# kevinzakka/mink

Hardware: AMD Instinct MI355X
Metric: IK solves/sec (whole node), Unitree G1 4 FrameTasks + box limits, batch 65536 (higher is better)
Workload: dtype f64

## Files before the change

### mink_amd/csrc/build.py

```python

import concurrent.futures
import json
import os
import re
import shutil
import subprocess
import sys
from typing import NamedTuple

HERE = os.path.dirname(os.path.abspath(__file__))
PKG = os.path.dirname(HERE)
_TAG = os.environ.get("MKH_BUILD_TAG", "")
LIB = os.path.join(PKG, f"libminkhip_{_TAG}.so" if _TAG else "libminkhip.so")
RESOURCES = os.path.join(PKG, f"kernel_resources_{_TAG}.json" if _TAG else "kernel_resources.json")
BUILD = os.path.join(HERE, f"_build_{_TAG}" if _TAG else "_build")
def _sources() -> list:
    fs = [os.path.join(HERE, f) for f in sorted(os.listdir(HERE))
          if f.endswith((".h", ".hip", ".py", ".inc")) and f not in ("tab_asm.inc", "__init__.py")]
    return fs + [os.path.join(HERE, "..", "..", "include", "minkhip.h")]


NTS = (8, 16, 24, 32, 44, 48, 64)
FEATS = (0, 16, 6, 8, 72, 88, 136, 30, 31, 256)
WOOD = ((16, 16), (24, 24), (32, 32), (44, 44), (48, 48))
W3 = ((44, 0),)
W3_WOOD = ((44, 44, 32), (44, 44, 48), (32, 32, 32), (32, 32, 48),
           (24, 24, 32), (24, 24, 48), (16, 16, 32), (16, 16, 48),
           (44, 44, 36), (44, 44, 52))
W3_WOOD_ONE_SHOT = ((44, 44, 32), (44, 44, 32, "w4"))
WOOD_FEATS = (32, 48, 33, 36, 52)
WOOD_ROWS = ((48, 48, 40),)


class Variant(NamedTuple):
    nt: int
    feat: int
    nr: int = 0
    w3: bool = False
    one_shot: bool = False
    w4 = False

    @property
    def name(self) -> str:
        return f"{self.nt}_{self.feat}" + (f"_r{self.nr}" if self.nr else "") + (("_w4" if self.w4 else "_w3") if self.w3 else "") + ("o" if self.one_shot else "")

    def translation_unit(self) -> str:
        defs = [f"MKH_NT {self.nt}"] + ([f"MKH_NR {self.nr}"] if self.nr else []) + [f"MKH_FEAT {self.feat}"]
        if self.w3:
            defs.append("MKH_W3 1")
            if self.w4:
                defs.append("MKH_W4P 1")
            elif self.nr and self.nt <= 24 and not self.one_shot:
                defs.append("MKH_W4 1")
        if self.one_shot:
            defs.append("MKH_ONE_SHOT 1")
        if self.name != f"{self.nt}_{self.feat}":
            defs.append(f"MKH_KERNEL_NAME ik_solve_kernel_{self.name}")
        return "// generated by build.py\n" + "".join(f"#define {d}\n" for d in defs) + f"""#include "../ik_kernel.h"
namespace mkh {{
void launch_{self.name}(int grid, int lds_bytes, hipStream_t stream, const DeviceProblem* P, const SolveArgs& a,
                      const TapArgs* taps) {{
  hipLaunchKernelGGL(ik_solve_kernel_{self.name}, dim3(grid), dim3(kWave), lds_bytes, stream, P, a, taps);
}}
}}  // namespace mkh
"""


class VariantW4(Variant):
    __slots__ = ()
    w4 = True


VARIANTS = tuple([Variant(nt, ft) for nt in NTS for ft in FEATS]
                 + [Variant(nt, ft, nr) for nt, nr in WOOD for ft in WOOD_FEATS]
                 + [Variant(nt, ft, nr) for nt, nr, ft in WOOD_ROWS]
                 + [Variant(nt, ft, w3=True) for nt, ft in W3]
                 + [Variant(nt, ft, nr, w3=True) for nt, nr, ft in W3_WOOD]
                 + [(VariantW4 if e[3:] == ("w4",) else Variant)(e[0], e[2], e[1], w3=True, one_shot=True) for e in W3_WOOD_ONE_SHOT])
FLAGS = ["--offload-arch=gfx950", "-O3", "-std=c++17", "-fPIC", "-Wno-unused-result", "-Wno-null-conversion"]
FLAGS += os.environ.get("MKH_EXTRA_FLAGS", "").split()
KERNEL_FLAGS = ["-mllvm", "-disable-machine-licm",
                "-Wno-inline-asm"]


def _hipcc() -> str:
    return shutil.which("hipcc") or "/opt/rocm/bin/hipcc"


def _stale() -> bool:
    if not os.path.exists(LIB) or not os.path.exists(RESOURCES) or not os.path.exists(BUILD_INFO):
        return True
    t = os.path.getmtime(LIB)
    return any(os.path.getmtime(p) > t for p in _sources()) \
        or not os.path.exists(os.path.join(HERE, "tab_asm.inc"))


def _deps(depfile: str) -> list:
    txt = open(depfile).read().replace("\\\n", " ")
    return [d for d in txt.split(":", 1)[1].split() if d]


def _obj_stale(src: str, obj: str, cmd_tag: str) -> bool:
    dep, tag = obj + ".d", obj + ".cmd"
    if not (os.path.exists(obj) and os.path.exists(dep) and os.path.exists(tag)) or open(tag).read() != cmd_tag:
        return True
    t = os.path.getmtime(obj)
    try:
        return any(os.path.getmtime(d) > t for d in [src] + _deps(dep))
    except OSError:
        return True


def _parse_resource_remarks(stderr: str) -> dict:
    out, cur = {}, None
    keys = {"VGPRs": "vgprs", "AGPRs": "agprs", "TotalSGPRs": "sgprs", "ScratchSize [bytes/lane]": "scratch_bytes_per_lane",
            "Occupancy [waves/SIMD]": "occupancy_waves_per_simd", "SGPRs Spill": "sgpr_spills", "VGPRs Spill": "vgpr_spills"}
    for m in re.finditer(r"remark:\s+([A-Za-z \[\]/]+): (\S+) \[-Rpass-analysis", stderr):
        k, v = m.group(1).strip(), m.group(2)
        if k == "Function Name":
            cur = out.setdefault(v, {})
        elif cur is not None and k in keys:
            cur[keys[k]] = int(v)
    return out


def _short_name(mangled: str) -> str:
    m = re.match(r"_ZN(?:3mkh|12_GLOBAL__N_1)(\d+)", mangled)
    if not m:
        return mangled
    n, a = int(m.group(1)), m.end()
    name, rest = mangled[a:a + n], mangled[a + n:]
    if rest.startswith("I"):
        args = re.match(r"I((?:L[ib]\d+E)+)E", rest)
        if args:
            name += "<" + ",".join(re.findall(r"L[ib](\d+)E", args.group(1))) + ">"
    return name


def _sha256(path: str) -> str:
    import hashlib
    h = hashlib.sha256()
    with open(path, "rb") as fh:
        for blk in iter(lambda: fh.read(1 << 20), b""):
            h.update(blk)
    return h.hexdigest()


def _device_code_sha256(obj: str) -> str:
    import hashlib
    import tempfile
    llvm = "/opt/rocm/lib/llvm/bin"
    try:
        with tempfile.TemporaryDirectory() as d:
            fat, co = os.path.join(d, "x.fatbin"), os.path.join(d, "x.co")
            subprocess.run([f"{llvm}/llvm-objcopy", f"--dump-section=.hip_fatbin={fat}", obj, os.path.join(d, "x.o")], check=True, capture_output=True)
            subprocess.run([f"{llvm}/clang-offload-bundler", "--unbundle", "--type=o", "--targets=hipv4-amdgcn-amd-amdhsa--gfx950",
                            f"--input={fat}", f"--output={co}"], check=True, capture_output=True)
            h = hashlib.sha256()
            for sec in (".text", ".rodata"):
                out = os.path.join(d, "sec.bin")
                subprocess.run([f"{llvm}/llvm-objcopy", "-O", "binary", f"--only-section={sec}", co, out], check=True, capture_output=True)
                with open(out, "rb") as fh:
                    h.update(fh.read())
            return h.hexdigest()
    except (OSError, subprocess.CalledProcessError):
        return _sha256(obj)


def _git_state() -> dict:
    root = os.path.dirname(PKG)
    try:
        head = subprocess.run(["git", "-C", root, "rev-parse", "HEAD"], capture_output=True, text=True, check=True).stdout.strip()
        dirty = subprocess.run(["git", "-C", root, "status", "--porcelain", "--", "mink_amd", "include"], capture_output=True,
                               text=True, check=True).stdout.strip() != ""
        return {"git_head": head, "git_dirty_sources": dirty}
    except (OSError, subprocess.CalledProcessError):
        return {"git_head": None, "git_dirty_sources": None}


BUILD_INFO = os.path.join(PKG, f"build_info_{_TAG}.json" if _TAG else "build_info.json")


def _write_resources(objs: list) -> None:
    table = {}
    for o in objs:
        path = o + ".res.json"
        if not os.path.exists(path):
            continue
        fns = json.load(open(path))
        kernels = {f: r for f, r in fns.items() if "ik_solve_kernel" in f or "ik_lane_kernel" in f or "_kernel" in _short_name(f)}
        callees = {f: r for f, r in fns.items() if f not in kernels}
        code = _device_code_sha256(o)
        for f, r in kernels.items():
            e = dict(r)
            e["code_sha256"] = code
            e["callees"] = {_short_name(c): cr for c, cr in callees.items()}
            e["vgpr_spills_with_callees"] = r.get("vgpr_spills", 0) + sum(cr.get("vgpr_spills", 0) for cr in callees.values())
            e["sgpr_spills_with_callees"] = r.get("sgpr_spills", 0) + sum(cr.get("sgpr_spills", 0) for cr in callees.values())
            table[_short_name(f)] = e
    with open(RESOURCES, "w") as fh:
        json.dump(table, fh, indent=0, sort_keys=True)
    info = {"library": os.path.basename(LIB), "library_sha256": _sha256(LIB)}
    info.update(_git_state())
    with open(BUILD_INFO, "w") as fh:
# ... 111 lines not shown
```

### mink_amd/csrc/ik_kernel.h

```cpp
#pragma once
#include "collide_dev.h"
#include "lds_layout.h"
#include "lie_dev.h"
#include "mkh_types.h"
#include "wave_ops.h"
#include "tab_asm.inc"
#include <utility>

#if defined(MKH_W4P) && !defined(MKH_W4)
#define MKH_W4 1
#endif
#if defined(MKH_W4)
#define MKH_TAB TabW4
#elif defined(MKH_W3)
#define MKH_TAB TabW3
#else
#define MKH_TAB Tab
#endif

#if defined(MKH_W3) || (defined(MKH_FEAT) && (MKH_FEAT & 8) && !(MKH_FEAT & 1) && !(MKH_FEAT & 64) && (!(MKH_FEAT & 128) || !defined(MKH_INLINE_136)))
#define MKH_CALLS 1
#endif

namespace mkh {
// ... 155 lines not shown
  const double2 a = o[0], b = o[1];
  ps.d = a.x; ps.sg = a.y; ps.x = b.x; ps.rn = b.y;
  if (FULL) {
    const double2 c = o[2];
    ps.lo = c.x; ps.hi = c.y;
  }
  double rowv = 0.0;
#ifdef MKH_W4P
  rowv = MKH_TAB<NT>::row_on_demand_1(ts, p0, p1, col, npiv, lds_addr(sPiv + kPivBuf));
#else
  if constexpr (MKH_TAB<NT>::kHist > 0) rowv = MKH_TAB<NT>::row_on_demand(ts, p0, p1, col, npiv);
#endif
  return (lane == col || lane >= nact) ? 0.0 : rowv;
}
template <int NT>
__device__ __forceinline__ void load_factor_column(typename MKH_TAB<NT>::Regs& ts, const double* sJ, const double* sDinv, int lane, int n_mu) {
  if constexpr (MKH_TAB<NT>::kHist > 0) MKH_TAB<NT>::load_gz(ts, lds_addr(sJ + (lane < NT ? lane : 0)), lds_addr(sDinv), n_mu);
}
#ifdef MKH_W4P
#define MKH_HS_PARAM , double* sHs
#define MKH_HS_ARG , sPiv + kPivBuf
#else
#define MKH_HS_PARAM
#define MKH_HS_ARG
#endif
template <int NT>
__device__ __forceinline__ void pivot_product(typename MKH_TAB<NT>::Regs& ts, QpLane& s, int k, bool reverse, int lane, double own,
                                              const PivotScalars& ps, double inv, int& npiv MKH_HS_PARAM) {
  const double sk = ps.sg;
  const double ck = s.sg * sk * own;
#ifdef MKH_W4P
  MKH_TAB<NT>::hist_push_1(ts, npiv, own);
  if (lane == k) reinterpret_cast<double2*>(sHs)[npiv] = double2{sk * sk, inv};
#else
  const double g = (sk * sk) * own * inv;
  if constexpr (MKH_TAB<NT>::kHist > 0) MKH_TAB<NT>::hist_push(ts, npiv, -g, own);
#endif
  ++npiv;
  if (lane == k) {
    s.D = -inv;
    s.sg = (reverse ? -sk : sk) * inv;
  } else {
    s.D = fma(-ck * inv, ck, s.D);
  }
}

constexpr bool kTapIsProf_t_xpos = false, kTapIsProf_t_xquat = false, kTapIsProf_t_frame_pose = false,
               kTapIsProf_t_subtree_com = false, kTapIsProf_t_task_e = false, kTapIsProf_t_task_J = false,
               kTapIsProf_t_H = false, kTapIsProf_t_c = false, kTapIsProf_t_box_lo = false, kTapIsProf_t_box_hi = false,
               kTapIsProf_t_coll_G = false, kTapIsProf_t_coll_h = false, kTapIsProf_t_qp_iters = true,
               kTapIsProf_t_cycles = true;


#ifdef MKH_NT
#ifdef MKH_DEBUG_ALL_TAPS
#define MKH_TAP(f) ((kTaps && tp) ? tp->f : nullptr)
#else
#define MKH_TAP(f) ((kTaps && tp && (!kWood || kTapIsProf_##f)) ? tp->f : nullptr)
#endif
#define MKH_CAT2(a, b, c) a##b##_##c
#define MKH_CAT(a, b, c) MKH_CAT2(a, b, c)
#ifndef MKH_KERNEL_NAME
#define MKH_KERNEL_NAME MKH_CAT(ik_solve_kernel_, MKH_NT, MKH_FEAT)
#endif

#ifdef MKH_MARKERS
#define MKH_MARK(name) asm volatile("; MKH_MARK " name)
#else
#define MKH_MARK(name) do {} while (0)
#endif

struct PreOut { int status, d_kind, d_k, d_body, d_qadr, conv; double mu_lane; V3 com_root; };
#ifdef MKH_CALLS
#ifdef MKH_ONE_SHOT
#define MKH_PRE_ATTR __attribute__((noinline, internal_linkage))
#else
#define MKH_PRE_ATTR __attribute__((noinline))
#endif
#ifdef MKH_CLOCKS
#define MKH_PRE_TC_PARAMS , long long* clk_row
#define MKH_PRE_TC_ARGS , (A.clk ? A.clk + (size_t)pb * 24 + 20 : nullptr)
#define MKH_PRE_TICK() do { if (clk_row) { *clk_row = __builtin_readcyclecounter(); ++clk_row; } asm volatile("" : "+v"(lane)); } while (0)
#define MKH_PRE_STOP(id) do { if (clk_row_stop == (id)) return PreOut{}; } while (0)
#else
#define MKH_PRE_TC_PARAMS
#define MKH_PRE_TC_ARGS
#define MKH_PRE_TICK() do { asm volatile("" : "+v"(lane)); } while (0)
#define MKH_PRE_STOP(id) do {} while (0)
#endif
#else
#define MKH_PRE_ATTR __forceinline__
#define MKH_PRE_TC_PARAMS , long long (&tc)[8], int& tci
#define MKH_PRE_TC_ARGS , tc, tci
#ifdef MKH_CLOCKS
#define MKH_PRE_TICK() do { tc[tci] = __builtin_readcyclecounter(); ++tci; asm volatile("" : "+v"(lane)); } while (0)
#else
#define MKH_PRE_TICK() do { if (MKH_TAP(t_cycles)) tc[tci] = __builtin_readcyclecounter(); ++tci; asm volatile("" : "+v"(lane)); } while (0)
#endif
#define MKH_PRE_STOP(id) do {} while (0)
#endif
#define MKH_GLOBAL __attribute__((address_space(1)))
#define MKH_CONSTANT __attribute__((address_space(4)))
struct PreView {
  const MKH_GLOBAL double *body_f, *jnt_f, *dof_f;
  const MKH_GLOBAL int32_t *body_i, *jnt_i, *dof_i;
  const MKH_GLOBAL FrameTaskDev* frame;
  int nbody, nv, nq, njnt, n_frame, n_posture, n_com, max_rows, n_jrows, prefetch, prefetch_w3, prefetch_w3w, wood_compact, prefetch_wc, n_rows_tap, nrounds, robot_root, n_hsel, jnt_pos_zero;
  __device__ __forceinline__ explicit PreView(const DeviceProblem* Pq) {
    const MKH_CONSTANT DeviceProblem* c = (const MKH_CONSTANT DeviceProblem*)Pq;
    body_f = (const MKH_GLOBAL double*)c->body_f; jnt_f = (const MKH_GLOBAL double*)c->jnt_f; dof_f = (const MKH_GLOBAL double*)c->dof_f;
    body_i = (const MKH_GLOBAL int32_t*)c->body_i; jnt_i = (const MKH_GLOBAL int32_t*)c->jnt_i; dof_i = (const MKH_GLOBAL int32_t*)c->dof_i;
    frame = (const MKH_GLOBAL FrameTaskDev*)c->frame;
    nbody = c->nbody; nv = c->nv; nq = c->nq; njnt = c->njnt; n_frame = c->n_frame; n_posture = c->n_posture; n_com = c->n_com;
    max_rows = c->max_rows; n_jrows = c->n_jrows; prefetch = c->prefetch; prefetch_w3 = c->prefetch_w3; prefetch_w3w = c->prefetch_w3w;
    wood_compact = c->wood_compact; prefetch_wc = c->prefetch_wc;
    n_rows_tap = c->n_rows_tap; nrounds = c->nrounds; robot_root = c->robot_root; n_hsel = c->n_hsel;
    jnt_pos_zero = c->jnt_pos_zero;
  }
};
template <class PT>
__device__ __forceinline__ bool kernel_prefetch(const PT& P0) {
  constexpr bool kWood = (MKH_FEAT & F_WOOD) != 0;
  constexpr bool kWoodRows = kWood && (MKH_FEAT & (F_COLL | F_DENSE)) != 0;
#if defined(MKH_W4P)
  (void)kWood; (void)kWoodRows; (void)P0;
  return false;
#elif defined(MKH_W3)
  return (kWood ? P0.prefetch_w3w : P0.prefetch_w3) != 0;
#else
  return ((kWoodRows || (kWood && P0.wood_compact != 0)) ? P0.prefetch_wc : P0.prefetch) != 0;
#endif
}
#ifdef MKH_NR
#define MKH_LAYOUT_NR MKH_NR
#else
#define MKH_LAYOUT_NR MKH_NT
#endif
#ifdef MKH_W3
#define MKH_LAYOUT_W3 true
#else
#define MKH_LAYOUT_W3 false
#endif
#ifdef MKH_W4P
#define kernel_lds_layout(P0) build_lds_layout_w4p(P0, MKH_LAYOUT_NR)
#else
#define kernel_lds_layout(P0) build_lds_layout(P0, MKH_NT, MKH_LAYOUT_NR, MKH_FEAT, MKH_LAYOUT_W3)
#endif
#ifdef MKH_W4P
#define MKH_PRE_RF_PARAM , int refetch, const SolveArgs* args_p
#define MKH_PRE_RF_ARG , (refac_in ? 1 : 0), (const SolveArgs*)A_p
#else
#define MKH_PRE_RF_PARAM
#define MKH_PRE_RF_ARG
#endif
__device__ MKH_PRE_ATTR PreOut pre_phases(const DeviceProblem* Pq, const TapArgs* tp, int pb, int oz, int off_q, int off_tgt,
                                          bool until, double pos_thr, double ori_thr MKH_PRE_RF_PARAM MKH_PRE_TC_PARAMS) {
  constexpr int FEAT = MKH_FEAT;
  constexpr bool kTaps = (FEAT & F_TAPS) != 0, kRel = (FEAT & F_REL) != 0, kCom = (FEAT & F_COM) != 0;
  constexpr bool kSteps = (FEAT & F_STEPS) != 0, kWood = (FEAT & F_WOOD) != 0;
  extern __shared__ __attribute__((aligned(16))) double smem[];
#if defined(MKH_CALLS) && defined(MKH_CLOCKS)
  const int clk_row_stop = clk_row ? (int)clk_row[-5] : 0;
#endif
#ifdef MKH_CALLS
  pb = uni(pb); oz = uni(oz); off_q = uni(off_q); off_tgt = uni(off_tgt);
  until = uni((int)until) != 0; pos_thr = uni(pos_thr); ori_thr = uni(ori_thr);
  Pq = reinterpret_cast<const DeviceProblem*>(uni((unsigned long long)reinterpret_cast<size_t>(Pq)));
  tp = reinterpret_cast<const TapArgs*>(uni((unsigned long long)reinterpret_cast<size_t>(tp)));
#endif
#ifdef MKH_CALLS
  const PreView P(Pq);
#else
  const DeviceProblem& P = *Pq;
#endif
  int lane = lane_id();
  const int ol = lane + oz;
  const int nbody = P.nbody, nv = P.nv;
  const LdsLayout L = kernel_lds_layout(P);
  double* const sq = smem + off_q;
  double* const sX = smem + L.X;
  const int XS = lds_even(nbody);
  double* const sJnt = smem + L.jnt;
  double* const sTgt = smem + off_tgt;
  double* const sTask = smem + L.task;
  double* const sDof = smem + L.dof;
  double* const sCom = smem + L.com;
  const bool is_body = lane < nbody;
  const bool is_dof = lane < nv;
  int status = 0;
#ifdef MKH_W4P
  if (uni(refetch) != 0) {
    typedef const __attribute__((address_space(1))) void* gptr_t;
    typedef __attribute__((address_space(3))) void* lptr_t;
    const MKH_CONSTANT SolveArgs& A = *(const MKH_CONSTANT SolveArgs*)uni((unsigned long long)reinterpret_cast<size_t>(args_p));
    wave_sync();
    const int ndq = 2 * P.nq, ndt = 2 * P.n_frame * 7;
    const char* gq = reinterpret_cast<const char*>(A.q + (size_t)pb * P.nq);
    for (int b0 = 0; b0 < ndq; b0 += kWave)
      if (b0 + lane < ndq)
        __builtin_amdgcn_global_load_lds((gptr_t)(gq + 4 * (b0 + lane)), (lptr_t)(reinterpret_cast<char*>(sq) + 4 * b0), 4, 0, 0);
    const char* gt = reinterpret_cast<const char*>(A.frame_targets + (size_t)pb * (ndt / 2));
    for (int b0 = 0; b0 < ndt; b0 += kWave)
      if (b0 + lane < ndt)
        __builtin_amdgcn_global_load_lds((gptr_t)(gt + 4 * (b0 + lane)), (lptr_t)(reinterpret_cast<char*>(sTgt) + 4 * b0), 4, 0, 0);
    asm volatile("s_waitcnt vmcnt(0)" ::: "memory");
    wave_sync();
  }
#endif
    V3 xp{0, 0, 0};
    Q4 xq{1, 0, 0, 0};
    int b_jadr = 0, b_jnum = 0, anc_lo = 0, anc_hi = 0;
    const bool jp_zero = kWood && P.jnt_pos_zero != 0;
    if (is_body) {
      anc_lo = P.body_i[BI_ANCPACK0 * 64 + ol];
      anc_hi = P.body_i[BI_ANCPACK1 * 64 + ol];
      const auto* bf = P.body_f + ol;
      xp = {bf[(BF_POS + 0) * 64], bf[(BF_POS + 1) * 64], bf[(BF_POS + 2) * 64]};
      xq = {bf[(BF_QUAT + 0) * 64], bf[(BF_QUAT + 1) * 64], bf[(BF_QUAT + 2) * 64], bf[(BF_QUAT + 3) * 64]};
      b_jadr = P.body_i[BI_JNTADR * 64 + ol];
      b_jnum = P.body_i[BI_JNTNUM * 64 + ol];
      for (int jn = 0; jn < b_jnum; ++jn) {
        const int j = b_jadr + jn;
        const int jt = P.jnt_i[j * JI_COUNT + JI_TYPE];
        const int qa = P.jnt_i[j * JI_COUNT + JI_QADR];
        const auto* jfp = P.jnt_f + j * JF_COUNT;
#ifdef MKH_W4P
        const auto* const jf = jfp;
#else
        const double jf[JF_COUNT] = {jfp[0], jfp[1], jfp[2], jfp[3], jfp[4], jfp[5], jfp[6]};
#endif
        if (jt == JNT_FREE) {
          xp = {sq[qa], sq[qa + 1], sq[qa + 2]};
          xq = qnormalize(Q4{sq[qa + 3], sq[qa + 4], sq[qa + 5], sq[qa + 6]});
        } else if (jt == JNT_SLIDE) {
          V3 ax{jf[JF_AXIS], jf[JF_AXIS + 1], jf[JF_AXIS + 2]};
          xp = xp + (sq[qa] - jf[JF_QPOS0]) * qrot(xq, ax);
        } else {
          V3 jp{jf[JF_POS], jf[JF_POS + 1], jf[JF_POS + 2]};
          Q4 qloc;
          if (jt == JNT_HINGE) {
            V3 ax{jf[JF_AXIS], jf[JF_AXIS + 1], jf[JF_AXIS + 2]};
            qloc = axis_angle(ax, sq[qa] - jf[JF_QPOS0]);
          } else {
            qloc = qnormalize(Q4{sq[qa], sq[qa + 1], sq[qa + 2], sq[qa + 3]});
          }
          V3 anchor = xp;
          if (!jp_zero) anchor = xp + qrot(xq, jp);
          xq = qmul(xq, qloc);
          xp = anchor;
          if (!jp_zero) xp = anchor - qrot(xq, jp);
        }
      }
    }
    for (int r = 0; r < P.nrounds; ++r) {
      wave_sync();
      if (is_body) {
        double* o = sX + lane;
        o[0] = xp.x; o[XS] = xp.y; o[2 * XS] = xp.z; o[3 * XS] = xq.w; o[4 * XS] = xq.x; o[5 * XS] = xq.y; o[6 * XS] = xq.z;
      }
      wave_sync();
      if (is_body) {
        const double* a = sX + (((r < 5) ? (anc_lo >> (6 * r)) : anc_hi) & 63);
        V3 ap{a[0], a[XS], a[2 * XS]};
        Q4 aq{a[3 * XS], a[4 * XS], a[5 * XS], a[6 * XS]};
        xp = ap + qrot(aq, xp);
        xq = qmul(aq, xq);
      }
    }
    xq = qnormalize(xq);
    wave_sync();
    if (is_body) {
      double* o = sX + lane;
      o[0] = xp.x; o[XS] = xp.y; o[2 * XS] = xp.z; o[3 * XS] = xq.w; o[4 * XS] = xq.x; o[5 * XS] = xq.y; o[6 * XS] = xq.z;
      if (MKH_TAP(t_xpos)) {
        double* t = MKH_TAP(t_xpos) + ((size_t)pb * nbody + lane) * 3;
        t[0] = xp.x; t[1] = xp.y; t[2] = xp.z;
      }
      if (MKH_TAP(t_xquat)) {
        double* t = MKH_TAP(t_xquat) + ((size_t)pb * nbody + lane) * 4;
        t[0] = xq.w; t[1] = xq.x; t[2] = xq.y; t[3] = xq.z;
      }
    }
    wave_sync();
    MKH_MARK("fk_done");
    MKH_PRE_TICK();
    MKH_PRE_STOP(1);
    if (is_body && b_jnum > 0) {
      if (b_jnum == 1) {
        const int j = b_jadr;
        const auto* jf = P.jnt_f + j * JF_COUNT;
        V3 ax = qrot(xq, V3{jf[JF_AXIS], jf[JF_AXIS + 1], jf[JF_AXIS + 2]});
        V3 an = xp;
        if (!jp_zero) an = xp + qrot(xq, V3{jf[JF_POS], jf[JF_POS + 1], jf[JF_POS + 2]});
        double* o = sJnt + j * 6;
        o[0] = ax.x; o[1] = ax.y; o[2] = ax.z; o[3] = an.x; o[4] = an.y; o[5] = an.z;
      } else {
        const double* a = sX + P.body_i[BI_PARENT * 64 + ol];
        const auto* bf = P.body_f + ol;
        V3 fp = V3{a[0], a[XS], a[2 * XS]} + qrot(Q4{a[3 * XS], a[4 * XS], a[5 * XS], a[6 * XS]},
                                            V3{bf[(BF_POS + 0) * 64], bf[(BF_POS + 1) * 64], bf[(BF_POS + 2) * 64]});
        Q4 fq = qmul(Q4{a[3 * XS], a[4 * XS], a[5 * XS], a[6 * XS]}, Q4{bf[(BF_QUAT + 0) * 64], bf[(BF_QUAT + 1) * 64],
                                                    bf[(BF_QUAT + 2) * 64], bf[(BF_QUAT + 3) * 64]});
        for (int jn = 0; jn < b_jnum; ++jn) {
          const int j = b_jadr + jn;
          const int jt = P.jnt_i[j * JI_COUNT + JI_TYPE];
          const int qa = P.jnt_i[j * JI_COUNT + JI_QADR];
          const auto* jf = P.jnt_f + j * JF_COUNT;
          V3 axl{jf[JF_AXIS], jf[JF_AXIS + 1], jf[JF_AXIS + 2]};
          V3 jp{jf[JF_POS], jf[JF_POS + 1], jf[JF_POS + 2]};
          V3 ax = qrot(fq, axl);
          V3 an = fp + qrot(fq, jp);
          double* o = sJnt + j * 6;
          o[0] = ax.x; o[1] = ax.y; o[2] = ax.z; o[3] = an.x; o[4] = an.y; o[5] = an.z;
          if (jt == JNT_SLIDE) {
            fp = fp + (sq[qa] - jf[JF_QPOS0]) * ax;
          } else if (jt == JNT_HINGE || jt == JNT_BALL) {
            Q4 qloc = (jt == JNT_HINGE) ? axis_angle(axl, sq[qa] - jf[JF_QPOS0])
                                        : qnormalize(Q4{sq[qa], sq[qa + 1], sq[qa + 2], sq[qa + 3]});
            fq = qmul(fq, qloc);
            fp = an - qrot(fq, jp);
          }
        }
      }
    }
    wave_sync();
    int d_kind = DOF_HINGE, d_k = 0, d_body = 0, d_qadr = -1;
    {
    V3 d_ang{0, 0, 0}, d_lin{0, 0, 0}, d_anchor{0, 0, 0};
    double q_dof = 0.0;
    const double r_lo = P.dof_f[DF_RANGE_LO * 64 + ol], r_hi = P.dof_f[DF_RANGE_HI * 64 + ol];
    if (is_dof) {
      const auto* di = P.dof_i + ol;
      const int d_jnt = di[DI_JNT * 64];
      d_kind = di[DI_KIND * 64];
      d_k = di[DI_K * 64];
      d_body = di[DI_BODY * 64];
      d_qadr = di[DI_QADR * 64];
      if (d_kind == DOF_HINGE) {
        const double* o = sJnt + d_jnt * 6;
        d_ang = {o[0], o[1], o[2]};
        d_anchor = {o[3], o[4], o[5]};
        q_dof = sq[d_qadr];
      } else if (d_kind == DOF_SLIDE) {
        const double* o = sJnt + d_jnt * 6;
        d_lin = {o[0], o[1], o[2]};
        q_dof = sq[d_qadr];
      } else if (d_kind == DOF_FREE_LIN) {
        d_lin = {d_k == 0 ? 1.0 : 0.0, d_k == 1 ? 1.0 : 0.0, d_k == 2 ? 1.0 : 0.0};
      } else {
        const double* xb = sX + d_body;
        M3 R = qmat(Q4{xb[3 * XS], xb[4 * XS], xb[5 * XS], xb[6 * XS]});
        d_ang = (d_k == 0) ? V3{R.m[0], R.m[3], R.m[6]}
                           : ((d_k == 1) ? V3{R.m[1], R.m[4], R.m[7]} : V3{R.m[2], R.m[5], R.m[8]});
        if (d_kind == DOF_FREE_ANG) {
          d_anchor = {xb[0], xb[XS], xb[2 * XS]};
        } else {
          const double* o = sJnt + d_jnt * 6;
          d_anchor = {o[3], o[4], o[5]};
        }
      }
    }
    {
      const bool ball0 = is_dof && d_kind == DOF_BALL && d_k == 0;
      const bool ranged = (is_dof && (d_kind == DOF_HINGE || d_kind == DOF_SLIDE)) || ball0;
      const double qc = ball0 ? sq[ball0 ? d_qadr : 0] : q_dof;
      const bool viol = ranged & ((qc < r_lo - 1e-6) | (qc > r_hi + 1e-6));
      if (__ballot(viol)) status |= 1;
    }
    if (is_dof) {
      double* o = sDof + lane * 10;
      o[0] = d_ang.x; o[1] = d_ang.y; o[2] = d_ang.z; o[3] = d_lin.x; o[4] = d_lin.y; o[5] = d_lin.z;
      o[6] = d_anchor.x; o[7] = d_anchor.y; o[8] = d_anchor.z; o[9] = q_dof;
    }
    }

    V3 com_root{0, 0, 0};
    if (kCom && P.n_com > 0) {
      V3 b_ipos{0, 0, 0};
      double b_mass = 0.0, b_stmass = 0.0;
      int b_last = 0, b_inrobot = 0;
      if (is_body) {
        const auto* bf = P.body_f + ol;
        b_ipos = {bf[(BF_IPOS + 0) * 64], bf[(BF_IPOS + 1) * 64], bf[(BF_IPOS + 2) * 64]};
        b_mass = bf[BF_MASS * 64];
        b_stmass = bf[BF_SUBTREEMASS * 64];
        b_last = P.body_i[BI_SUBTREE_LAST * 64 + ol];
        b_inrobot = P.body_i[BI_IN_ROBOT * 64 + ol];
      }
      V3 xi = xp + qrot(xq, b_ipos);
      const double m = (is_body && b_inrobot) ? b_mass : 0.0;
      double sx = m * xi.x, sy = m * xi.y, sz = m * xi.z;
#pragma unroll
      for (int o = 1; o < 64; o <<= 1) {
        double tx = __shfl_up(sx, o), ty = __shfl_up(sy, o), tz = __shfl_up(sz, o);
        if (lane >= o) { sx += tx; sy += ty; sz += tz; }
      }
      const int hi_l = is_body ? b_last : 0, lo_l = lane - 1;
      double ex = __shfl(sx, hi_l), ey = __shfl(sy, hi_l), ez = __shfl(sz, hi_l);
      double bx = __shfl(sx, lo_l < 0 ? 0 : lo_l), by = __shfl(sy, lo_l < 0 ? 0 : lo_l),
             bz = __shfl(sz, lo_l < 0 ? 0 : lo_l);
      if (lane == 0) { bx = 0; by = 0; bz = 0; }
      V3 cs = xi;
      if (b_stmass >= 1e-15) {
        const double im = fast_rcp(b_stmass);
        cs = {(ex - bx) * im, (ey - by) * im, (ez - bz) * im};
      }
      if (is_body) {
        double* o = sCom + lane * 4;
        o[0] = cs.x; o[1] = cs.y; o[2] = cs.z; o[3] = b_stmass;
      }
      wave_sync();
      const double* cr = sCom + P.robot_root * 4;
      com_root = {cr[0], cr[1], cr[2]};
      if (MKH_TAP(t_subtree_com) && lane < 3) MKH_TAP(t_subtree_com)[(size_t)pb * 3 + lane] = cr[lane];
    }

    MKH_MARK("axes_done");
    MKH_PRE_TICK();
    MKH_PRE_STOP(2);
    double mu_lane = 0.0;
    bool conv_lane = true;
    if (lane < P.n_frame) {
      const auto& ft = P.frame[lane];
      const double* xb = sX + ft.body;
      SE3 F;
      Q4 bq{xb[3 * XS], xb[4 * XS], xb[5 * XS], xb[6 * XS]};
      F.p = V3{xb[0], xb[XS], xb[2 * XS]} + qrot(bq, V3{ft.lpos[0], ft.lpos[1], ft.lpos[2]});
      F.q = qmul(bq, Q4{ft.lquat[0], ft.lquat[1], ft.lquat[2], ft.lquat[3]});
      const double* tg = sTgt + lane * 7;
      SE3 Tt{Q4{tg[0], tg[1], tg[2], tg[3]}, V3{tg[4], tg[5], tg[6]}};
      double* o = sTask + lane * 64;
      V3 ev, ew;
      double Jm[9], Qm[9];
      bool ident;
      double eth = 0.0;
      const double* const eth_p = kWood ? &eth : nullptr;
#ifdef MKH_W4P
      {
        const M3 Rf0 = qmat(F.q);
#pragma unroll
        for (int i = 0; i < 9; ++i) o[18 + i] = Rf0.m[i];
        o[27] = F.p.x; o[28] = F.p.y; o[29] = F.p.z;
      }
#endif
      if (!(kRel && ft.relative)) {
        se3_log(se3_mul(se3_inv(F), Tt), ev, ew, eth);
        se3_ljacinv(ev, ew, eth_p, Jm, Qm, ident);
      } else {
        const double* xr = sX + ft.root_body;
        Q4 rq0{xr[3 * XS], xr[4 * XS], xr[5 * XS], xr[6 * XS]};
        SE3 Rt;
        Rt.p = V3{xr[0], xr[XS], xr[2 * XS]} + qrot(rq0, V3{ft.root_lpos[0], ft.root_lpos[1], ft.root_lpos[2]});
        Rt.q = qmul(rq0, Q4{ft.root_lquat[0], ft.root_lquat[1], ft.root_lquat[2], ft.root_lquat[3]});
        const SE3 Tfr = se3_mul(se3_inv(Rt), F);
        se3_log(se3_mul(se3_inv(Tt), Tfr), ev, ew, eth);
        se3_ljacinv(-1.0 * ev, -1.0 * ew, eth_p, Jm, Qm, ident);
        const SE3 Trf = se3_inv(Tfr);
        const M3 Rr = qmat(Rt.q), Rrf = qmat(Trf.q);
#pragma unroll
        for (int i = 0; i < 9; ++i) { o[36 + i] = Rr.m[i]; o[48 + i] = Rrf.m[i]; }
        o[45] = Rt.p.x; o[46] = Rt.p.y; o[47] = Rt.p.z;
        o[57] = Trf.p.x; o[58] = Trf.p.y; o[59] = Trf.p.z;
        if (MKH_TAP(t_frame_pose)) {
          double* t = MKH_TAP(t_frame_pose) + ((size_t)pb * P.n_frame + lane) * 7;
          t[0] = Tfr.q.w; t[1] = Tfr.q.x; t[2] = Tfr.q.y; t[3] = Tfr.q.z; t[4] = Tfr.p.x; t[5] = Tfr.p.y; t[6] = Tfr.p.z;
        }
      }
#ifdef MKH_W4P
#pragma unroll
      for (int i = 0; i < 9; ++i) { o[i] = Jm[i]; o[9 + i] = Qm[i]; }
#else
      M3 Rf = qmat(F.q);
#pragma unroll
      for (int i = 0; i < 9; ++i) { o[i] = Jm[i]; o[9 + i] = Qm[i]; o[18 + i] = Rf.m[i]; }
      o[27] = F.p.x; o[28] = F.p.y; o[29] = F.p.z;
#endif
      const double e6[6] = {ev.x, ev.y, ev.z, ew.x, ew.y, ew.z};
      double ss = 0.0;
#pragma unroll
      for (int r = 0; r < 6; ++r) {
        const double we = ft.cost[r] * (-ft.gain * e6[r]);
        o[30 + r] = we;
        ss += we * we;
        if (MKH_TAP(t_task_e)) MKH_TAP(t_task_e)[(size_t)pb * P.n_rows_tap + ft.row0 + r] = e6[r];
      }
      mu_lane = ft.lm_damping * ss;
      if (kSteps && until) {
        const double pt = pos_thr, ot = ori_thr;
        conv_lane = (!(ft.rowmask & 7) || dot(ev, ev) <= pt * pt) && (!(ft.rowmask & 56) || dot(ew, ew) <= ot * ot);
      }
      if (MKH_TAP(t_frame_pose) && !(kRel && ft.relative)) {
        double* t = MKH_TAP(t_frame_pose) + ((size_t)pb * P.n_frame + lane) * 7;
        t[0] = F.q.w; t[1] = F.q.x; t[2] = F.q.y; t[3] = F.q.z; t[4] = F.p.x; t[5] = F.p.y; t[6] = F.p.z;
      }
    }
  PreOut po;
  po.status = status; po.d_kind = d_kind; po.d_k = d_k; po.d_body = d_body; po.d_qadr = d_qadr;
  po.conv = conv_lane ? 1 : 0; po.mu_lane = mu_lane; po.com_root = com_root;
  return po;
}

template <bool kRel>
__device__ __forceinline__ void frame_column_fn(const double* sTask, const double* sDof, int t, int k, uint64_t mask,
                                                uint64_t rmask, bool rel, double (&Jt)[6]) {
    const double* o = sTask + t * 64;
    const double* kd = sDof + k * 10;
    const V3 d_ang{kd[0], kd[1], kd[2]}, d_lin{kd[3], kd[4], kd[5]}, d_anchor{kd[6], kd[7], kd[8]};
    V3 a{0, 0, 0}, w{0, 0, 0};
    if ((mask >> k) & 1) {
      V3 pf{o[27], o[28], o[29]};
      V3 jp = d_lin + cross(d_ang, pf - d_anchor);
      M3 Rf;
#pragma unroll
      for (int i = 0; i < 9; ++i) Rf.m[i] = o[18 + i];
      a = mulT(Rf, jp); w = mulT(Rf, d_ang);
    }
    double sign = -1.0;
    if (kRel && rel) {
      sign = 1.0;
      if ((rmask >> k) & 1) {
        V3 pr{o[45], o[46], o[47]};
        V3 jp = d_lin + cross(d_ang, pr - d_anchor);
        M3 Rr, Rrf;
#pragma unroll
        for (int i = 0; i < 9; ++i) { Rr.m[i] = o[36 + i]; Rrf.m[i] = o[48 + i]; }
        V3 ar = mulT(Rr, jp), wr = mulT(Rr, d_ang);
        V3 Rw = mul(Rrf, wr);
        a = a - (mul(Rrf, ar) + cross(V3{o[57], o[58], o[59]}, Rw));
        w = w - Rw;
      }
    }
    const double wv[3] = {w.x, w.y, w.z};
    double y[3], z3[3];
#pragma unroll
    for (int r = 0; r < 3; ++r) y[r] = o[3 * r] * wv[0] + o[3 * r + 1] * wv[1] + o[3 * r + 2] * wv[2];
    const double av[3] = {a.x, a.y, a.z};
#pragma unroll
    for (int r = 0; r < 3; ++r)
      z3[r] = av[r] - (o[9 + 3 * r] * y[0] + o[9 + 3 * r + 1] * y[1] + o[9 + 3 * r + 2] * y[2]);
#pragma unroll
    for (int r = 0; r < 3; ++r) {
      Jt[r] = sign * (o[3 * r] * z3[0] + o[3 * r + 1] * z3[1] + o[3 * r + 2] * z3[2]);
      Jt[3 + r] = sign * y[r];
    }
  }

struct DirectPairs { double Jp[6]; int p_task, p_dof; };
__device__ MKH_PRE_ATTR DirectPairs direct_pairs(const DeviceProblem* Pq) {
  constexpr bool kRel = (MKH_FEAT & F_REL) != 0;
  extern __shared__ __attribute__((aligned(16))) double smem[];
#ifdef MKH_CALLS
  Pq = reinterpret_cast<const DeviceProblem*>(uni((unsigned long long)reinterpret_cast<size_t>(Pq)));
  const MKH_CONSTANT DeviceProblem& P = *(const MKH_CONSTANT DeviceProblem*)Pq;
  const MKH_GLOBAL FrameTaskDev* const frames = (const MKH_GLOBAL FrameTaskDev*)P.frame;
#else
  const DeviceProblem& P = *Pq;
  const FrameTaskDev* const frames = P.frame;
#endif
  const int lane = lane_id();
  const LdsLayout L = kernel_lds_layout(P);
  DirectPairs dp{{0, 0, 0, 0, 0, 0}, -1, 0};
  if (lane < P.n_dpairs) {
    dp.p_task = P.dpair_task[lane]; dp.p_dof = P.dpair_dof[lane];
    const auto& ft = frames[dp.p_task];
    const bool rel = kRel && ft.relative != 0;
    double Jt[6];
    frame_column_fn<kRel>(smem + L.task, smem + L.dof, dp.p_task, dp.p_dof, ft.dof_mask, rel ? ft.root_mask : 0ull, rel, Jt);
#pragma unroll
    for (int r = 0; r < 6; ++r) dp.Jp[r] = ft.cost[r] * Jt[r];
  }
  return dp;
}


#if (MKH_FEAT & 32)
struct WoodOut { double hdiag, dsq, x, D, rown; int status, clamp; };

template <int SRC, int O0, int O1>
__device__ __forceinline__ void wood_store_pivot(unsigned addr, double inv, double om) {
  static_assert(SRC >= 0 && SRC < kWave && O0 >= 0 && O0 < 256 && O1 >= 0 && O1 < 256, "lane / ds_write2 offsets");
  unsigned long long sv;
  asm volatile("s_mov_b64 %[sv], exec\n\ts_lshl_b64 exec, 1, %[src]\n\tds_write2_b64 %[a], %[x], %[y] offset0:%[o0] offset1:%[o1]\n\t"
               "s_mov_b64 exec, %[sv]"
               : [sv] "=&s"(sv) : [a] "v"(addr), [x] "v"(inv), [y] "v"(om), [src] "n"(SRC), [o0] "n"(O0), [o1] "n"(O1) : "memory", "scc");
}

struct WoodRefine { bool on; int nv; double lo, hi, zfree, dsq, sqdg, zsq; };
template <int K, bool DUAL>
__device__ __forceinline__ void wood_eliminate(int n_mu, int NR, int lane, double* sJ, double* sS, int SP, const double* sW,
                                               double* sRow, double* sDinv, double& ssq, double& quad, double& zw, int& status,
                                               const WoodRefine& rf, int& clamp, double& beta) {
  const unsigned plane_off = (unsigned)(lane & 15);
  if constexpr (!DUAL) {
    const int my_c = lane - NR;
    const bool is_s = my_c >= 0 && my_c < n_mu;
    double z[K];
    {
      const double* src = sJ + lane;
      int stride = NR;
      bool live = lane < NR;
      if (is_s) { src = sS + my_c * SP; stride = 1; live = true; }
#pragma unroll
      for (int r = 0; r < K; ++r) z[r] = (live && r < n_mu) ? src[r * stride] : 0.0;
    }
    double ws = is_s ? sW[my_c] : 0.0;
    {
      double q = 0.0;
#pragma unroll
      for (int r = 0; r < K; ++r) q = fma(z[r], z[r], q);
      if (lane < NR) sJ[n_mu * NR + lane] = q;
    }
    double* const sOm = sDinv + kMuOm;
    int n_mu_s = uni(n_mu);
    unsigned dinv_addr = lds_addr(sDinv);
    asm volatile("" : "+v"(dinv_addr));
#pragma nounroll
    for (int pass = 0;; ++pass) {
      quad = 0.0; zw = 0.0;
      asm volatile("" : "+s"(n_mu_s));
      static_for<K>([&](auto rc) {
        constexpr int r = decltype(rc)::value;
        if (r < n_mu_s) {
          const double d = readlane_f64(z[r], NR + r), om = readlane_f64(ws, NR + r);
          const double p0 = bperm_f64(z[r], NR + (int)plane_off);
          const double p1 = (K > 16) ? bperm_f64(z[r], (NR + 16 + (int)plane_off) & 63) : 0.0;
          if (lane < NR) sJ[r * NR + lane] = z[r];
          const double inv = fast_rcp(d);
          wood_store_pivot<(MKH_NT + r) % kWave, r, kMuOm + r>(dinv_addr, inv, ws);
          const double zi = z[r] * inv;
          quad = fma(z[r], zi, quad);
          zw = fma(om, zi, zw);
          WoodElim<r, K>::step(z, p0, p1, -zi);
          ws = fma(-zi, om, ws);
        }
      });
      if (lane < n_mu && !(sDinv[lane] > 0.0)) status |= 4;
      if (pass == 1 || !rf.on) break;
#ifdef MKH_W4P
      double rc = rf.zsq, rd = rf.dsq, rh = rf.sqdg;
      asm volatile("" : "+v"(rc), "+v"(rd), "+v"(rh));
      double rf_zfree = rc * (rd * rd), rf_sqdg = rh * rd, rf_zsq = rc * rd;
      asm volatile("" : "+v"(rf_zfree), "+v"(rf_sqdg), "+v"(rf_zsq));
      const double x0 = rf_zfree - rd * zw;
#else
      const double x0 = rf.zfree - rf.dsq * zw;
// ... 1822 lines not shown
```

### mink_amd/csrc/lie_dev.h

```cpp
#pragma once
#include <hip/hip_runtime.h>

namespace mkh {

__device__ __forceinline__ double fast_rcp(double d) {
  double r = __builtin_amdgcn_rcp(d);
  r = fma(fma(-d, r, 1.0), r, r);
  r = fma(fma(-d, r, 1.0), r, r);
  return r;
}

struct V3 { double x, y, z; };
struct Q4 { double w, x, y, z; };
struct M3 { double m[9]; };

__device__ __forceinline__ V3 v3(double x, double y, double z) { return V3{x, y, z}; }
__device__ __forceinline__ V3 operator+(V3 a, V3 b) { return {a.x + b.x, a.y + b.y, a.z + b.z}; }
__device__ __forceinline__ V3 operator-(V3 a, V3 b) { return {a.x - b.x, a.y - b.y, a.z - b.z}; }
__device__ __forceinline__ V3 operator*(double s, V3 a) { return {s * a.x, s * a.y, s * a.z}; }
__device__ __forceinline__ double dot(V3 a, V3 b) { return a.x * b.x + a.y * b.y + a.z * b.z; }
__device__ __forceinline__ V3 cross(V3 a, V3 b) {
  return {a.y * b.z - a.z * b.y, a.z * b.x - a.x * b.z, a.x * b.y - a.y * b.x};
}

__device__ __forceinline__ Q4 qmul(Q4 a, Q4 b) {
  return {a.w * b.w - a.x * b.x - a.y * b.y - a.z * b.z,
          a.w * b.x + a.x * b.w + a.y * b.z - a.z * b.y,
          a.w * b.y - a.x * b.z + a.y * b.w + a.z * b.x,
          a.w * b.z + a.x * b.y - a.y * b.x + a.z * b.w};
}
__device__ __forceinline__ Q4 qconj(Q4 a) { return {a.w, -a.x, -a.y, -a.z}; }
__device__ __forceinline__ Q4 qnormalize(Q4 q) {
  double n = sqrt(q.w * q.w + q.x * q.x + q.y * q.y + q.z * q.z);
  if (n < 1e-15) return {1.0, 0.0, 0.0, 0.0};
  double inv = fast_rcp(n);
  return {q.w * inv, q.x * inv, q.y * inv, q.z * inv};
}
__device__ __forceinline__ M3 qmat(Q4 q) {
  M3 r;
  double q00 = q.w * q.w, q01 = q.w * q.x, q02 = q.w * q.y, q03 = q.w * q.z;
  double q11 = q.x * q.x, q12 = q.x * q.y, q13 = q.x * q.z;
  double q22 = q.y * q.y, q23 = q.y * q.z, q33 = q.z * q.z;
  r.m[0] = q00 + q11 - q22 - q33; r.m[4] = q00 - q11 + q22 - q33; r.m[8] = q00 - q11 - q22 + q33;
  r.m[1] = 2 * (q12 - q03); r.m[2] = 2 * (q13 + q02); r.m[3] = 2 * (q12 + q03);
  r.m[5] = 2 * (q23 - q01); r.m[6] = 2 * (q13 - q02); r.m[7] = 2 * (q23 + q01);
  return r;
}
__device__ __forceinline__ V3 mul(const M3& R, V3 v) {
  return {R.m[0] * v.x + R.m[1] * v.y + R.m[2] * v.z,
          R.m[3] * v.x + R.m[4] * v.y + R.m[5] * v.z,
          R.m[6] * v.x + R.m[7] * v.y + R.m[8] * v.z};
}
__device__ __forceinline__ V3 mulT(const M3& R, V3 v) {
  return {R.m[0] * v.x + R.m[3] * v.y + R.m[6] * v.z,
          R.m[1] * v.x + R.m[4] * v.y + R.m[7] * v.z,
          R.m[2] * v.x + R.m[5] * v.y + R.m[8] * v.z};
}
__device__ __forceinline__ V3 qrot(Q4 q, V3 v) {
  V3 u{q.x, q.y, q.z};
  V3 t = 2.0 * cross(u, v);
  return v + q.w * t + cross(u, t);
}
__device__ __forceinline__ void sincos_cw(double x, double* sn, double* cs) {
  const double n = rint(x * 0.63661977236758134308);
  double r = fma(-n, 1.57079632679489655800e+00, x);
  r = fma(-n, 6.12323399573676603587e-17, r);
  r = fma(-n, -1.49738490485916983e-33, r);
  const double z = r * r;
  const double ps = fma(z, fma(z, fma(z, fma(z, fma(z, 1.58969099521155010221e-10, -2.50507602534068634195e-08),
                                               2.75573137070700676789e-06), -1.98412698298579493134e-04),
                              8.33333333332248946124e-03), -1.66666666666666324348e-01);
  const double s0 = fma(r * z, ps, r);
  const double pc = fma(z, fma(z, fma(z, fma(z, fma(z, -1.13596475577881948265e-11, 2.08757232129817482790e-09),
                                               -2.75573143513906633035e-07), 2.48015872894767294178e-05),
                              -1.38888888888741095749e-03), 4.16666666666666019037e-02);
  const double c0 = fma(z * z, pc, fma(-0.5, z, 1.0));
  const int q = ((int)n) & 3;
  const double sv = (q & 1) ? c0 : s0;
  const double cv = (q & 1) ? s0 : c0;
  *sn = (q & 2) ? -sv : sv;
  *cs = ((q + 1) & 2) ? -cv : cv;
}

__device__ __forceinline__ Q4 axis_angle(V3 axis, double angle) {
  double s, c;
  sincos_cw(0.5 * angle, &s, &c);
  return {c, axis.x * s, axis.y * s, axis.z * s};
}

__device__ __forceinline__ V3 so3_log(Q4 q) {
  const double w = q.w;
  const double norm_sq = q.x * q.x + q.y * q.y + q.z * q.z;
  double factor;
  if (norm_sq < 1e-10) {
    const double iw = fast_rcp(w);
    factor = 2.0 * iw - 2.0 / 3.0 * norm_sq * (iw * iw * iw);
  } else {
    const double nrm = sqrt(norm_sq);
    if (fabs(w) < 1e-10) {
      factor = (w > 0.0 ? 1.0 : -1.0) * M_PI * fast_rcp(nrm);
    } else {
      factor = 2.0 * atan2(w < 0 ? -nrm : nrm, fabs(w)) * fast_rcp(nrm);
    }
  }
  return {factor * q.x, factor * q.y, factor * q.z};
}

__device__ __forceinline__ Q4 so3_exp(V3 w) {
  const double th2 = w.x * w.x + w.y * w.y + w.z * w.z;
  double re, im;
  if (th2 < 1e-10) {
    const double th4 = th2 * th2;
    re = 1.0 - th2 / 8.0 + th4 / 384.0;
    im = 0.5 - th2 / 48.0 + th4 / 3840.0;
  } else {
    const double th = sqrt(th2);
    double s;
    sincos_cw(0.5 * th, &s, &re);
    im = s / th;
  }
  return {re, im * w.x, im * w.y, im * w.z};
}

__device__ __forceinline__ V3 quat2vel(Q4 q) {
  double ax[3] = {q.x, q.y, q.z};
  const double sn = sqrt(ax[0] * ax[0] + ax[1] * ax[1] + ax[2] * ax[2]);
  if (sn < 1e-15) { ax[0] = 1; ax[1] = 0; ax[2] = 0; } else { ax[0] /= sn; ax[1] /= sn; ax[2] /= sn; }
  double sp = 2.0 * atan2(sn, q.w);
  if (sp > M_PI) sp -= 2.0 * M_PI;
  return V3{ax[0] * sp, ax[1] * sp, ax[2] * sp};
}

struct SE3 { Q4 q; V3 p; };
__device__ __forceinline__ SE3 se3_mul(SE3 a, SE3 b) { return {qmul(a.q, b.q), qrot(a.q, b.p) + a.p}; }
__device__ __forceinline__ SE3 se3_inv(SE3 a) { Q4 qi = qconj(a.q); return {qi, -1.0 * qrot(qi, a.p)}; }

__device__ __forceinline__ void se3_log(SE3 T, V3& v, V3& omega, double& th) {
  omega = so3_log(T.q);
  const double th2 = dot(omega, omega);
  double k;
  th = 0.0;
  if (th2 < 1e-10) {
    k = 1.0 / 12.0;
  } else {
    th = sqrt(th2);
    double s, c;
    sincos_cw(0.5 * th, &s, &c);
    k = (1.0 - th * c * fast_rcp(2.0 * s)) * fast_rcp(th2);
  }
  V3 wt = cross(omega, T.p);
  v = T.p - 0.5 * wt + k * cross(omega, wt);
}
__device__ __forceinline__ void se3_log(SE3 T, V3& v, V3& omega) { double th; se3_log(T, v, omega, th); }

__device__ __forceinline__ void se3_ljacinv(V3 v, V3 w, const double* th_in, double* J, double* Q, bool& ident) {
  const double th2 = dot(w, w);
  ident = th2 < 1e-10;
  if (ident) {
#pragma unroll
    for (int i = 0; i < 9; ++i) { J[i] = (i % 4 == 0) ? 1.0 : 0.0; Q[i] = 0.0; }
    return;
  }
  const double th = th_in ? *th_in : sqrt(th2);
  double s, c;
  sincos_cw(th, &s, &c);
  const double ith2 = fast_rcp(th2), ith = th * ith2, ith4 = ith2 * ith2;
  const double A = ith2 * (1.0 - (th * s * fast_rcp(2.0 * (1.0 - c))));
  const double Bc = (th - s) * (ith2 * ith);
  const double Cc = (1.0 - th2 * 0.5 - c) * ith4;
  const double Dc = (2.0 * th - 3.0 * s + th * c) * (0.5 * ith4 * ith);
  const double wv[3] = {w.x, w.y, w.z}, vv[3] = {v.x, v.y, v.z};
  const double sv = dot(w, v);
  const V3 u = cross(v, w);
  const V3 wu = cross(w, u);
  const V3 sk = (0.5 + 2.0 * Cc * th2) * v + (-(Bc + 3.0 * Cc) * sv) * w + (-Cc) * wu;
  const double skv[3] = {sk.x, sk.y, sk.z};
  const double dgq = -2.0 * Bc * sv + 2.0 * Dc * sv * th2;
#pragma unroll
  for (int i = 0; i < 3; ++i)
#pragma unroll
    for (int j = 0; j < 3; ++j) {
      double sym = Bc * (vv[i] * wv[j] + wv[i] * vv[j]) - 2.0 * Dc * sv * (wv[i] * wv[j]);
      double w2 = wv[i] * wv[j];
      double skw = 0.0, skq = 0.0;
      if (i != j) {
        const int k = 3 - i - j;
        const double sg = ((j - i + 3) % 3 == 1) ? -1.0 : 1.0;
        skw = sg * wv[k];
        skq = sg * skv[k];
      } else {
        sym += dgq;
        w2 -= th2;
      }
      J[3 * i + j] = ((i == j) ? 1.0 : 0.0) - 0.5 * skw + A * w2;
      Q[3 * i + j] = sym + skq;
    }
}
__device__ __forceinline__ void se3_ljacinv(V3 v, V3 w, double* J, double* Q, bool& ident) {
  se3_ljacinv(v, w, nullptr, J, Q, ident);
}

}
```

Baseline: 129.3 million.

## Pair lanes per frame task to split sincos work, use SGPR-loaded polynomial constants

For the W4P variant, each frame task with at most 8 frames is now handled by two lanes. The high partner lane computes sincos(th) while the low lane computes sincos(th/2), and the result is passed back via a DPP row shift. This removes one serial sincos from each active lane's critical path by using idle lanes. It also adds inline-asm FMAs that load 64-bit polynomial constants through VCC scalar moves instead of VGPR literal materialisation, which is meant to cut register use and instruction count, at the cost of clobbering VCC and relying on the DPP pattern being correct.

```diff
diff --git a/mink_amd/csrc/build.py b/mink_amd/csrc/build.py
--- a/mink_amd/csrc/build.py
+++ b/mink_amd/csrc/build.py
@@ -50,6 +50,7 @@
             defs.append("MKH_W3 1")
             if self.w4:
                 defs.append("MKH_W4P 1")
+                defs.append("MKH_SCONST 1")
             elif self.nr and self.nt <= 24 and not self.one_shot:
                 defs.append("MKH_W4 1")
         if self.one_shot:
diff --git a/mink_amd/csrc/ik_kernel.h b/mink_amd/csrc/ik_kernel.h
--- a/mink_amd/csrc/ik_kernel.h
+++ b/mink_amd/csrc/ik_kernel.h
@@ -331,6 +331,30 @@
 #else
 #define MKH_PRE_RF_PARAM
 #define MKH_PRE_RF_ARG
+#endif
+#ifdef MKH_W4P
+__device__ __forceinline__ void se3_log_paired(SE3 T, V3& v, V3& omega, double& th, bool pair, bool hi, double (&sc2)[2]) {
+  omega = so3_log(T.q);
+  const double th2 = dot(omega, omega);
+  double k;
+  th = 0.0;
+  if (th2 < 1e-10) {
+    k = 1.0 / 12.0;
+  } else {
+    th = sqrt(th2);
+    double s, c;
+    sincos_cw(hi ? th : 0.5 * th, &s, &c);
+    if (pair) {
+      sc2[0] = dpp_f64<0x108>(s);
+      sc2[1] = dpp_f64<0x108>(c);
+    } else {
+      sincos_cw(th, &sc2[0], &sc2[1]);
+    }
+    k = (1.0 - th * c * fast_rcp(2.0 * s)) * fast_rcp(th2);
+  }
+  V3 wt = cross(omega, T.p);
+  v = T.p - 0.5 * wt + k * cross(omega, wt);
+}
 #endif
 __device__ MKH_PRE_ATTR PreOut pre_phases(const DeviceProblem* Pq, const TapArgs* tp, int pb, int oz, int off_q, int off_tgt,
                                           bool until, double pos_thr, double ori_thr MKH_PRE_RF_PARAM MKH_PRE_TC_PARAMS) {
@@ -599,23 +623,33 @@
     MKH_PRE_STOP(2);
     double mu_lane = 0.0;
     bool conv_lane = true;
+#ifdef MKH_W4P
+    static_assert(!kRel, "the partner lanes store nothing: the RelativeFrameTask branch below is not guarded for them");
+    const bool pair = P.n_frame <= 8;
+    const int tl = pair ? (lane & 7) : lane;
+    const bool hi = pair && lane >= 8;
+    if (lane < (pair ? 16 : P.n_frame) && tl < P.n_frame) {
+#else
+    constexpr bool hi = false;
+    const int tl = lane;
     if (lane < P.n_frame) {
-      const auto& ft = P.frame[lane];
+#endif
+      const auto& ft = P.frame[tl];
       const double* xb = sX + ft.body;
       SE3 F;
       Q4 bq{xb[3 * XS], xb[4 * XS], xb[5 * XS], xb[6 * XS]};
       F.p = V3{xb[0], xb[XS], xb[2 * XS]} + qrot(bq, V3{ft.lpos[0], ft.lpos[1], ft.lpos[2]});
       F.q = qmul(bq, Q4{ft.lquat[0], ft.lquat[1], ft.lquat[2], ft.lquat[3]});
-      const double* tg = sTgt + lane * 7;
+      const double* tg = sTgt + tl * 7;
       SE3 Tt{Q4{tg[0], tg[1], tg[2], tg[3]}, V3{tg[4], tg[5], tg[6]}};
-      double* o = sTask + lane * 64;
+      double* o = sTask + tl * 64;
       V3 ev, ew;
       double Jm[9], Qm[9];
       bool ident;
       double eth = 0.0;
       const double* const eth_p = kWood ? &eth : nullptr;
 #ifdef MKH_W4P
-      {
+      if (!hi) {
         const M3 Rf0 = qmat(F.q);
 #pragma unroll
         for (int i = 0; i < 9; ++i) o[18 + i] = Rf0.m[i];
@@ -623,8 +657,14 @@
       }
 #endif
       if (!(kRel && ft.relative)) {
+#ifdef MKH_W4P
+        double sc2[2];
+        se3_log_paired(se3_mul(se3_inv(F), Tt), ev, ew, eth, pair, hi, sc2);
+        se3_ljacinv(ev, ew, eth_p, Jm, Qm, ident, sc2);
+#else
         se3_log(se3_mul(se3_inv(F), Tt), ev, ew, eth);
         se3_ljacinv(ev, ew, eth_p, Jm, Qm, ident);
+#endif
       } else {
         const double* xr = sX + ft.root_body;
         Q4 rq0{xr[3 * XS], xr[4 * XS], xr[5 * XS], xr[6 * XS]};
@@ -646,8 +686,10 @@
         }
       }
 #ifdef MKH_W4P
-#pragma unroll
-      for (int i = 0; i < 9; ++i) { o[i] = Jm[i]; o[9 + i] = Qm[i]; }
+      if (!hi) {
+#pragma unroll
+        for (int i = 0; i < 9; ++i) { o[i] = Jm[i]; o[9 + i] = Qm[i]; }
+      }
 #else
       M3 Rf = qmat(F.q);
 #pragma unroll
@@ -659,17 +701,17 @@
 #pragma unroll
       for (int r = 0; r < 6; ++r) {
         const double we = ft.cost[r] * (-ft.gain * e6[r]);
-        o[30 + r] = we;
+        if (!hi) o[30 + r] = we;
         ss += we * we;
-        if (MKH_TAP(t_task_e)) MKH_TAP(t_task_e)[(size_t)pb * P.n_rows_tap + ft.row0 + r] = e6[r];
-      }
-      mu_lane = ft.lm_damping * ss;
-      if (kSteps && until) {
+        if (!hi && MKH_TAP(t_task_e)) MKH_TAP(t_task_e)[(size_t)pb * P.n_rows_tap + ft.row0 + r] = e6[r];
+      }
+      if (!hi) mu_lane = ft.lm_damping * ss;
+      if (kSteps && until && !hi) {
         const double pt = pos_thr, ot = ori_thr;
         conv_lane = (!(ft.rowmask & 7) || dot(ev, ev) <= pt * pt) && (!(ft.rowmask & 56) || dot(ew, ew) <= ot * ot);
       }
-      if (MKH_TAP(t_frame_pose) && !(kRel && ft.relative)) {
-        double* t = MKH_TAP(t_frame_pose) + ((size_t)pb * P.n_frame + lane) * 7;
+      if (!hi && MKH_TAP(t_frame_pose) && !(kRel && ft.relative)) {
+        double* t = MKH_TAP(t_frame_pose) + ((size_t)pb * P.n_frame + tl) * 7;
         t[0] = F.q.w; t[1] = F.q.x; t[2] = F.q.y; t[3] = F.q.z; t[4] = F.p.x; t[5] = F.p.y; t[6] = F.p.z;
       }
     }
diff --git a/mink_amd/csrc/lie_dev.h b/mink_amd/csrc/lie_dev.h
--- a/mink_amd/csrc/lie_dev.h
+++ b/mink_amd/csrc/lie_dev.h
@@ -9,6 +9,28 @@
   r = fma(fma(-d, r, 1.0), r, r);
   return r;
 }
+
+#ifdef MKH_SCONST
+constexpr unsigned sc_lo(double c) { return (unsigned)(__builtin_bit_cast(unsigned long long, c) & 0xffffffffull); }
+constexpr unsigned sc_hi(double c) { return (unsigned)(__builtin_bit_cast(unsigned long long, c) >> 32); }
+template <unsigned kLo, unsigned kHi>
+__device__ __forceinline__ double fma_sc(double a, double b) {
+  double r;
+  asm("s_mov_b32 vcc_lo, %3\n\ts_mov_b32 vcc_hi, %4\n\tv_fma_f64 %0, %1, %2, vcc" : "=v"(r) : "v"(a), "v"(b), "n"(kLo), "n"(kHi) : "vcc");
+  return r;
+}
+template <unsigned kLo, unsigned kHi>
+__device__ __forceinline__ double fnma_sc(double n, double r0) {
+  double r;
+  asm("s_mov_b32 vcc_lo, %3\n\ts_mov_b32 vcc_hi, %4\n\tv_fma_f64 %0, -%1, vcc, %2" : "=v"(r) : "v"(n), "v"(r0), "n"(kLo), "n"(kHi) : "vcc");
+  return r;
+}
+#define MKH_FMA_SC(a, b, C) fma_sc<sc_lo(C), sc_hi(C)>((a), (b))
+#define MKH_FNMA_SC(n, C, r) fnma_sc<sc_lo(C), sc_hi(C)>((n), (r))
+#else
+#define MKH_FMA_SC(a, b, C) fma((a), (b), (C))
+#define MKH_FNMA_SC(n, C, r) fma(-(n), (C), (r))
+#endif
 
 struct V3 { double x, y, z; };
 struct Q4 { double w, x, y, z; };
@@ -63,17 +85,21 @@
 }
 __device__ __forceinline__ void sincos_cw(double x, double* sn, double* cs) {
   const double n = rint(x * 0.63661977236758134308);
-  double r = fma(-n, 1.57079632679489655800e+00, x);
-  r = fma(-n, 6.12323399573676603587e-17, r);
-  r = fma(-n, -1.49738490485916983e-33, r);
+  double r = MKH_FNMA_SC(n, 1.57079632679489655800e+00, x);
+  r = MKH_FNMA_SC(n, 6.12323399573676603587e-17, r);
+  r = MKH_FNMA_SC(n, -1.49738490485916983e-33, r);
   const double z = r * r;
-  const double ps = fma(z, fma(z, fma(z, fma(z, fma(z, 1.58969099521155010221e-10, -2.50507602534068634195e-08),
-                                               2.75573137070700676789e-06), -1.98412698298579493134e-04),
-                              8.33333333332248946124e-03), -1.66666666666666324348e-01);
+  double ps = MKH_FMA_SC(z, 1.58969099521155010221e-10, -2.50507602534068634195e-08);
+  ps = MKH_FMA_SC(z, ps, 2.75573137070700676789e-06);
+  ps = MKH_FMA_SC(z, ps, -1.98412698298579493134e-04);
+  ps = MKH_FMA_SC(z, ps, 8.33333333332248946124e-03);
+  ps = MKH_FMA_SC(z, ps, -1.66666666666666324348e-01);
   const double s0 = fma(r * z, ps, r);
-  const double pc = fma(z, fma(z, fma(z, fma(z, fma(z, -1.13596475577881948265e-11, 2.08757232129817482790e-09),
-                                               -2.75573143513906633035e-07), 2.48015872894767294178e-05),
-                              -1.38888888888741095749e-03), 4.16666666666666019037e-02);
+  double pc = MKH_FMA_SC(z, -1.13596475577881948265e-11, 2.08757232129817482790e-09);
+  pc = MKH_FMA_SC(z, pc, -2.75573143513906633035e-07);
+  pc = MKH_FMA_SC(z, pc, 2.48015872894767294178e-05);
+  pc = MKH_FMA_SC(z, pc, -1.38888888888741095749e-03);
+  pc = MKH_FMA_SC(z, pc, 4.16666666666666019037e-02);
   const double c0 = fma(z * z, pc, fma(-0.5, z, 1.0));
   const int q = ((int)n) & 3;
   const double sv = (q & 1) ? c0 : s0;
@@ -153,7 +179,8 @@
 }
 __device__ __forceinline__ void se3_log(SE3 T, V3& v, V3& omega) { double th; se3_log(T, v, omega, th); }
 
-__device__ __forceinline__ void se3_ljacinv(V3 v, V3 w, const double* th_in, double* J, double* Q, bool& ident) {
+__device__ __forceinline__ void se3_ljacinv(V3 v, V3 w, const double* th_in, double* J, double* Q, bool& ident,
+                                            const double* sc_in = nullptr) {
   const double th2 = dot(w, w);
   ident = th2 < 1e-10;
   if (ident) {
@@ -163,7 +190,7 @@
   }
   const double th = th_in ? *th_in : sqrt(th2);
   double s, c;
-  sincos_cw(th, &s, &c);
+  if (sc_in) { s = sc_in[0]; c = sc_in[1]; } else sincos_cw(th, &s, &c);
   const double ith2 = fast_rcp(th2), ith = th * ith2, ith4 = ith2 * ith2;
   const double A = ith2 * (1.0 - (th * s * fast_rcp(2.0 * (1.0 - c))));
   const double Bc = (th - s) * (ith2 * ith);
```

New measurement: 129.0 million. No clear change (-0.2%).
